# mims-harvard/Raindrop

Measured on AMD Instinct MI355X. Metric: samples/sec fwd+bwd, P19 34-sensor batch=256; % HBM roofline on msg-pass kernel, higher is better.
Workload: dtype f32

## Files before the change

include/raindrop_hip_debug.h:

```cpp
#ifndef RAINDROP_HIP_DEBUG_H
#define RAINDROP_HIP_DEBUG_H

#ifdef __cplusplus
extern "C" {
#endif

void rd_debug_set_stamps(void* device_u64);
void rd_debug_set_rowgemm_stamps(void* device_u64);
void rd_debug_set_attn_stamps(void* device_u64);
void rd_debug_set_gemm_stamps(void* device_u64);
void rd_debug_set_encfuse_stamps(void* device_u64);
void rd_debug_set_head_stamps(void* device_u64);
void rd_debug_set_attnfuse_stamps(void* device_u64);
void rd_debug_ifetch_probe(void* ticks_device_u64, void* scratch_64_floats, void* stream);
void rd_debug_set_splitk_want(int workgroups);

#ifdef __cplusplus
}
#endif
#endif
```

raindrop_amd/csrc/rd_attnfuse.hip:

```cpp
#include <stdlib.h>

#include "rd_common.h"
#include "rd_plan.h"
#include "rd_rng.h"

namespace rd {
namespace {

typedef __bf16 bf8 __attribute__((ext_vector_type(8)));
typedef __bf16 bf4 __attribute__((ext_vector_type(4)));
typedef short sh4 __attribute__((ext_vector_type(4)));
typedef short sh8 __attribute__((ext_vector_type(8)));

constexpr int TS = 64;
constexpr int LDT = TS;
__device__ __forceinline__ int tsw(int row) { return (row & 3) | (((row >> 3) & 1) << 2); }
__device__ __forceinline__ int tofs(int row, int col) { return row * LDT + ((((col >> 3) ^ tsw(row)) & 7) << 3) + (col & 7); }
constexpr int AF_WV = 8, AF_THR = 64 * AF_WV;

struct FAttnArgs {
  const float* x;
  const __bf16* wf;
  const __bf16* wb;
  const float* bias;
  float* out; float* lse;
  const float* dout; const float* ds1; float* dx;
  __bf16* xt; __bf16* dt;
  const int32_t* plan;
  int T, B, D, H, hd;
  float scale, p_drop; uint64_t seed; uint32_t site; const uint64_t* seed_cell;
  int one;
  unsigned long long* stamps;
};
static unsigned long long* g_af_stamps = nullptr;
#define AFSTAMP(i)                                                                                  \
  do {                                                                                              \
    if (a.stamps && blockIdx.x == 0 && threadIdx.x == 0) a.stamps[(i)] = clock64();                 \
  } while (0)

__device__ __forceinline__ float g16_max(float v) {
#define RD_ROR(v, n) __builtin_bit_cast(float, __builtin_amdgcn_update_dpp(0, __builtin_bit_cast(int, v), 0x120 + (n), 0xf, 0xf, false))
  v = fmaxf(v, RD_ROR(v, 8)); v = fmaxf(v, RD_ROR(v, 4)); v = fmaxf(v, RD_ROR(v, 2)); v = fmaxf(v, RD_ROR(v, 1));
  return v;
}
__device__ __forceinline__ float g16_sum(float v) {
  v += RD_ROR(v, 8); v += RD_ROR(v, 4); v += RD_ROR(v, 2); v += RD_ROR(v, 1);
#undef RD_ROR
  return v;
}

__device__ __forceinline__ bf8 frag_n(const __bf16* P, int ld, int row0, int k0, int lane) {
  return *reinterpret_cast<const bf8*>(P + (row0 + (lane & 15)) * ld + k0 + 8 * (lane >> 4));
}
__device__ __forceinline__ bf8 frag_t(const __bf16* P, int ld, int k0, int col0, int lane) {
  const int i = lane & 15, G = lane >> 4;
  const __bf16* src = P + (k0 + 8 * G + (i >> 2)) * ld + col0 + 4 * (i & 3);
  const sh4 lo = __builtin_amdgcn_ds_read_tr16_b64_v4i16((sh4 __attribute__((address_space(3)))*)(src));
  const sh4 hi = __builtin_amdgcn_ds_read_tr16_b64_v4i16((sh4 __attribute__((address_space(3)))*)(src + 4 * ld));
  const sh8 o = {lo[0], lo[1], lo[2], lo[3], hi[0], hi[1], hi[2], hi[3]};
  return __builtin_bit_cast(bf8, o);
}
__device__ __forceinline__ bf8 frag_ns(const __bf16* P, int row0, int k0, int lane) {
  return *reinterpret_cast<const bf8*>(P + tofs(row0 + (lane & 15), k0 + 8 * (lane >> 4)));
}
__device__ __forceinline__ bf8 frag_ts(const __bf16* P, int k0, int col0, int lane) {
  const int i = lane & 15, G = lane >> 4;
  const int row = k0 + 8 * G + (i >> 2), col = col0 + 4 * (i & 3);
  const __bf16* src = P + tofs(row, col);
  const sh4 lo = __builtin_amdgcn_ds_read_tr16_b64_v4i16((sh4 __attribute__((address_space(3)))*)(src));
  const sh4 hi = __builtin_amdgcn_ds_read_tr16_b64_v4i16((sh4 __attribute__((address_space(3)))*)(src + 4 * LDT));
  const sh8 o = {lo[0], lo[1], lo[2], lo[3], hi[0], hi[1], hi[2], hi[3]};
  return __builtin_bit_cast(bf8, o);
}
template <int NT, bool AT, bool BT, bool ASW, bool BSW>
__device__ __forceinline__ void mma_b16(f32x4 (&acc)[NT], const __bf16* Ah, const __bf16* Al, int lda, int a0, const __bf16* Bh,
                                        const __bf16* Bl, int ldb, int b0, int KK, int lane, bool one) {
  auto fa = [&](const __bf16* P, int k0) {
    if (ASW) return AT ? frag_ts(P, k0, a0, lane) : frag_ns(P, a0, k0, lane);
    return AT ? frag_t(P, lda, k0, a0, lane) : frag_n(P, lda, a0, k0, lane);
  };
  auto fb = [&](const __bf16* P, int k0, int j) {
    if (BSW) return BT ? frag_ts(P, k0, b0 + 16 * j, lane) : frag_ns(P, b0 + 16 * j, k0, lane);
    return BT ? frag_t(P, ldb, k0, b0 + 16 * j, lane) : frag_n(P, ldb, b0 + 16 * j, k0, lane);
  };
  if (!one) {
#pragma unroll
    for (int k0 = 0; k0 < KK; k0 += 32) {
      const bf8 ah = fa(Ah, k0);
      const bf8 al = fa(Al, k0);
      bf8 bh[NT], bl[NT];
#pragma unroll
      for (int j = 0; j < NT; ++j) { bh[j] = fb(Bh, k0, j); bl[j] = fb(Bl, k0, j); }
#pragma unroll
      for (int j = 0; j < NT; ++j) acc[j] = __builtin_amdgcn_mfma_f32_16x16x32_bf16(al, bh[j], acc[j], 0, 0, 0);
#pragma unroll
      for (int j = 0; j < NT; ++j) acc[j] = __builtin_amdgcn_mfma_f32_16x16x32_bf16(ah, bl[j], acc[j], 0, 0, 0);
#pragma unroll
      for (int j = 0; j < NT; ++j) acc[j] = __builtin_amdgcn_mfma_f32_16x16x32_bf16(ah, bh[j], acc[j], 0, 0, 0);
    }
  } else {
#pragma unroll
    for (int k0 = 0; k0 < KK; k0 += 32) {
      const bf8 ah = fa(Ah, k0);
#pragma unroll
      for (int j = 0; j < NT; ++j) {
        const bf8 bh = fb(Bh, k0, j);
        acc[j] = __builtin_amdgcn_mfma_f32_16x16x32_bf16(ah, bh, acc[j], 0, 0, 0);
      }
    }
  }
}

__device__ __forceinline__ void split4(const float (&v)[4], bf4& hi, bf4& lo) {
#pragma unroll
  for (int r = 0; r < 4; ++r) { hi[r] = (__bf16)v[r]; lo[r] = (__bf16)(v[r] - (float)hi[r]); }
}
__device__ __forceinline__ void store_t4(__bf16* Ph, __bf16* Pl, int row, int col4, const float (&v)[4]) {
  bf4 hi, lo;
  split4(v, hi, lo);
  const int o = tofs(row, col4);
  *reinterpret_cast<bf4*>(Ph + o) = hi;
  *reinterpret_cast<bf4*>(Pl + o) = lo;
}

__device__ __forceinline__ uint64_t attn_quad(int bh, int T, int q, int key) { return ((uint64_t)bh * T + key) * ((T + 3) >> 2) + (q >> 2); }
__device__ __forceinline__ void attn_keep4(float (&k4)[4], uint64_t seed, uint32_t site, int bh, int T, int q0, int key, float p, float inv_keep) {
  const float4 u = uniform4(seed, site, attn_quad(bh, T, q0, key));
  k4[0] = u.x >= p ? inv_keep : 0.f; k4[1] = u.y >= p ? inv_keep : 0.f;
  k4[2] = u.z >= p ? inv_keep : 0.f; k4[3] = u.w >= p ? inv_keep : 0.f;
}

template <int KCX>
struct XRows { float4 v[(TS * 8 * KCX) / AF_THR]; };

template <int KCX>
__device__ __forceinline__ void x_request(XRows<KCX>& r, const float* x, long row0, int Tv, int D, int tid) {
  constexpr int kq = 8 * KCX, NIT = (TS * kq) / AF_THR;
  static_assert((TS * kq) % AF_THR == 0, "x tile must divide over the workgroup");
#pragma unroll
  for (int it = 0; it < NIT; ++it) {
    const int i = tid + it * AF_THR;
    const int rr = i / kq, k = 4 * (i - rr * kq);
    r.v[it] = *reinterpret_cast<const float4*>(x + (row0 + min(rr, Tv - 1)) * D + min(k, D - 4));
  }
}
template <int KCX>
__device__ __forceinline__ void x_store(const XRows<KCX>& r, __bf16* Xh, __bf16* Xl, int Tv, int D, int tid) {
  constexpr int kq = 8 * KCX, NIT = (TS * kq) / AF_THR, LDX = 32 * KCX + 16;
#pragma unroll
  for (int it = 0; it < NIT; ++it) {
    const int i = tid + it * AF_THR;
    const int rr = i / kq, k = 4 * (i - rr * kq);
    const bool ok = rr < Tv && k < D;
    const float v[4] = {ok ? r.v[it].x : 0.f, ok ? r.v[it].y : 0.f, ok ? r.v[it].z : 0.f, ok ? r.v[it].w : 0.f};
    bf4 hi, lo;
    split4(v, hi, lo);
    *reinterpret_cast<bf4*>(Xh + rr * LDX + k) = hi;
    *reinterpret_cast<bf4*>(Xl + rr * LDX + k) = lo;
  }
}

template <int KCX>
struct QkvPanel { bf8 h[2][KCX], l[2][KCX]; float bs[2]; };

template <int NTH, int KCX>
__device__ __forceinline__ void qkv_request(QkvPanel<KCX>& p, const __bf16* wf_h, const float* bias, int D, int hd, int h, int wave, int lane) {
  constexpr int NCT3 = 3 * NTH;
  static_assert(NCT3 <= 2 * AF_WV, "two column tiles per wave");
#pragma unroll
  for (int s = 0; s < 2; ++s) {
    const int ct = min(wave + AF_WV * s, NCT3 - 1);
    const __bf16* t = wf_h + (size_t)ct * (KCX * 2 * 512) + lane * 8;
#pragma unroll
    for (int kc = 0; kc < KCX; ++kc) {
      p.h[s][kc] = *reinterpret_cast<const bf8*>(t + (kc * 2 + 0) * 512);
      p.l[s][kc] = *reinterpret_cast<const bf8*>(t + (kc * 2 + 1) * 512);
    }
    const int whc = ct / NTH, cl = 16 * (ct - whc * NTH) + (lane & 15);
    p.bs[s] = bias[whc * D + h * hd + min(cl, hd - 1)];
  }
}

template <int NTH, int KCX>
__device__ __forceinline__ void qkv_project(const QkvPanel<KCX>& p, const __bf16* Xh, const __bf16* Xl, int hd, int Tv, __bf16* Tp, int wave,
                                            int lane, bool one) {
  constexpr int NCT3 = 3 * NTH, HDP = 32 * ((16 * NTH + 31) / 32), LDX = 32 * KCX + 16;
  const bool two = wave + AF_WV < NCT3;
  const int aoff = (lane & 15) * LDX + 8 * (lane >> 4);
  f32x4 acc[2][4];
#pragma unroll
  for (int s = 0; s < 2; ++s)
#pragma unroll
    for (int rt = 0; rt < 4; ++rt) acc[s][rt] = (f32x4){0.f, 0.f, 0.f, 0.f};
  if (!one) {
#pragma unroll
    for (int kc = 0; kc < KCX; ++kc) {
      bf8 ah[4], al[4];
#pragma unroll
      for (int rt = 0; rt < 4; ++rt) {
        ah[rt] = *reinterpret_cast<const bf8*>(Xh + rt * 16 * LDX + aoff + kc * 32);
        al[rt] = *reinterpret_cast<const bf8*>(Xl + rt * 16 * LDX + aoff + kc * 32);
      }
#pragma unroll
      for (int s = 0; s < 2; ++s)
#pragma unroll
        for (int rt = 0; rt < 4; ++rt) acc[s][rt] = __builtin_amdgcn_mfma_f32_16x16x32_bf16(al[rt], p.h[s][kc], acc[s][rt], 0, 0, 0);
#pragma unroll
      for (int s = 0; s < 2; ++s)
#pragma unroll
        for (int rt = 0; rt < 4; ++rt) acc[s][rt] = __builtin_amdgcn_mfma_f32_16x16x32_bf16(ah[rt], p.l[s][kc], acc[s][rt], 0, 0, 0);
#pragma unroll
      for (int s = 0; s < 2; ++s)
#pragma unroll
        for (int rt = 0; rt < 4; ++rt) acc[s][rt] = __builtin_amdgcn_mfma_f32_16x16x32_bf16(ah[rt], p.h[s][kc], acc[s][rt], 0, 0, 0);
    }
  } else {
#pragma unroll
    for (int kc = 0; kc < KCX; ++kc) {
#pragma unroll
      for (int rt = 0; rt < 4; ++rt) {
        const bf8 ah = *reinterpret_cast<const bf8*>(Xh + rt * 16 * LDX + aoff + kc * 32);
#pragma unroll
        for (int s = 0; s < 2; ++s) acc[s][rt] = __builtin_amdgcn_mfma_f32_16x16x32_bf16(ah, p.h[s][kc], acc[s][rt], 0, 0, 0);
      }
    }
  }
#pragma unroll
  for (int s = 0; s < 2; ++s) {
    if (s == 1 && !two) break;
    const int ct = wave + AF_WV * s;
    const int whc = ct / NTH, cl = 16 * (ct - whc * NTH) + (lane & 15);
    __bf16* Ph = Tp + (size_t)(whc * 2) * HDP * LDT;
    __bf16* Pl = Ph + (size_t)HDP * LDT;
    const bool cok = cl < hd;
#pragma unroll
    for (int rt = 0; rt < 4; ++rt) {
      const int r0 = 16 * rt + 4 * (lane >> 4);
      float v[4];
#pragma unroll
      for (int r = 0; r < 4; ++r) v[r] = (cok && r0 + r < Tv) ? acc[s][rt][r] + p.bs[s] : 0.f;
      store_t4(Ph, Pl, cl, r0, v);
    }
  }
}

template <int NTH>
__device__ __forceinline__ void zero_pad_rows(__bf16* Tp, int tid) {
  constexpr int HDP = 32 * ((16 * NTH + 31) / 32), PADR = HDP - 16 * NTH;
  if (PADR == 0) return;
  constexpr int Q8 = LDT / 4;
  for (int i = tid; i < 6 * PADR * Q8; i += AF_THR) {
    const int pl = i / (PADR * Q8), rem = i - pl * (PADR * Q8);
    const int rr = rem / Q8, q = rem - rr * Q8;
    bf4 z;
#pragma unroll
    for (int c = 0; c < 4; ++c) z[c] = (__bf16)0.f;
    *reinterpret_cast<bf4*>(Tp + ((size_t)pl * HDP + 16 * NTH + rr) * LDT + 4 * q) = z;
  }
}

template <int NTH, int KCX, bool ONE>
__global__ __launch_bounds__(AF_THR) void k_attn_fwd_fused(FAttnArgs a) {
  extern __shared__ __attribute__((aligned(16))) unsigned char fsm[];
  RD_TOUCH_CODE(ONE ? RD_TL_ATTN_FWD_B : RD_TL_ATTN_FWD);
  constexpr int HDP = 32 * ((16 * NTH + 31) / 32), LDX = 32 * KCX + 16, NA = (NTH + 1) / 2;
  constexpr int LDO = 16 * NTH + 4;
  __bf16* Xh = reinterpret_cast<__bf16*>(fsm);
  __bf16* Xl = Xh + TS * LDX;
  __bf16* Tp = Xl + TS * LDX;
  __bf16 *Qh = Tp, *Ql = Qh + HDP * LDT, *Kh = Ql + HDP * LDT, *Kl = Kh + HDP * LDT, *Vh = Kl + HDP * LDT, *Vl = Vh + HDP * LDT;
  float* mxs = reinterpret_cast<float*>(Vl + HDP * LDT);
  float* sms = mxs + 2 * TS;
  __bf16 *Ph = Qh, *Pl = Ql;
  float* ost = reinterpret_cast<float*>(Kh);
  static_assert(HDP >= TS, "P^T must fit inside the Q^T plane");
  static_assert((size_t)TS * LDO * 4 <= (size_t)2 * HDP * LDT * 2, "output stage must fit inside the K^T planes");
  const int tid = threadIdx.x, lane = tid & 63, wave = __builtin_amdgcn_readfirstlane(tid >> 6), wq = wave & 3, wh = wave >> 2;
  const int b = blockIdx.x;
  const int Tv = __builtin_amdgcn_readfirstlane(a.plan[plan::len_base(a.B) + b]);
  if (Tv <= 0) return;
  const long row0 = __builtin_amdgcn_readfirstlane(a.plan[plan::off_base() + b]);
  uint64_t seedv = a.seed;
  XRows<KCX> xr;
  x_request<KCX>(xr, a.x, row0, Tv, a.D, tid);
  QkvPanel<KCX> pan;
  qkv_request<NTH, KCX>(pan, a.wf, a.bias, a.D, a.hd, 0, wave, lane);
  __builtin_amdgcn_sched_barrier(0);
  if (a.p_drop > 0.f && a.seed_cell) seedv += load_uniform_u64(a.seed_cell);
  zero_pad_rows<NTH>(Tp, tid);
  AFSTAMP(0);
  x_store<KCX>(xr, Xh, Xl, Tv, a.D, tid);
  AFSTAMP(1);
  lds_barrier();
  AFSTAMP(2);
  const float inv_keep = 1.0f / (1.0f - a.p_drop);
  constexpr bool one = ONE;
  const int qr0 = wq * 16 + 4 * (lane >> 4);
  for (int h = 0; h < a.H; ++h) {
    const int bh = b * a.H + h;
    if (h > 0) zero_pad_rows<NTH>(Tp, tid);
    qkv_project<NTH, KCX>(pan, Xh, Xl, a.hd, Tv, Tp, wave, lane, one);
    __builtin_amdgcn_sched_barrier(0);
    {
      const int hn = h + 1 < a.H ? h + 1 : 0;
      qkv_request<NTH, KCX>(pan, a.wf + (size_t)hn * (3 * NTH * KCX * 2 * 512), a.bias, a.D, a.hd, hn, wave, lane);
    }
    __builtin_amdgcn_sched_barrier(0);
    AFSTAMP(3 + 8 * h);
    lds_barrier();
    AFSTAMP(4 + 8 * h);
    float kp[2][4];
#pragma unroll
    for (int j = 0; j < 2; ++j)
      attn_keep4(kp[j], seedv, a.site, bh, a.T, qr0, min(16 * (2 * wh + j) + (lane & 15), a.T - 1), a.p_drop, inv_keep);
    f32x4 s[2];
#pragma unroll
    for (int j = 0; j < 2; ++j) s[j] = (f32x4){0.f, 0.f, 0.f, 0.f};
    mma_b16<2, true, true, true, true>(s, Qh, Ql, LDT, wq * 16, Kh, Kl, LDT, 32 * wh, HDP, lane, one);
    float mx[4] = {-INFINITY, -INFINITY, -INFINITY, -INFINITY};
#pragma unroll
    for (int j = 0; j < 2; ++j) {
      const int key = 16 * (2 * wh + j) + (lane & 15);
      const bool dead = key >= Tv;
#pragma unroll
      for (int r = 0; r < 4; ++r) {
        s[j][r] = dead ? -INFINITY : s[j][r] * a.scale;
        mx[r] = fmaxf(mx[r], s[j][r]);
      }
    }
#pragma unroll
    for (int r = 0; r < 4; ++r) {
      mx[r] = g16_max(mx[r]);
      if ((lane & 15) == 0) mxs[wh * TS + qr0 + r] = mx[r];
    }
    AFSTAMP(5 + 8 * h);
    lds_barrier();
    float m_i[4], rsum[4] = {0.f, 0.f, 0.f, 0.f};
#pragma unroll
    for (int r = 0; r < 4; ++r) m_i[r] = fmaxf(mxs[qr0 + r], mxs[TS + qr0 + r]);
#pragma unroll
    for (int j = 0; j < 2; ++j) {
      const int key = 16 * (2 * wh + j) + (lane & 15);
      float pv[4];
#pragma unroll
      for (int r = 0; r < 4; ++r) {
        const float p = (s[j][r] == -INFINITY) ? 0.f : __expf(s[j][r] - m_i[r]);
        rsum[r] += p;
        pv[r] = p * kp[j][r];
      }
      store_t4(Ph, Pl, key, qr0, pv);
    }
#pragma unroll
    for (int r = 0; r < 4; ++r) {
      rsum[r] = g16_sum(rsum[r]);
      if ((lane & 15) == 0) sms[wh * TS + qr0 + r] = rsum[r];
    }
    AFSTAMP(6 + 8 * h);
    lds_barrier();
    AFSTAMP(7 + 8 * h);
    float l_i[4];
#pragma unroll
    for (int r = 0; r < 4; ++r) l_i[r] = sms[qr0 + r] + sms[TS + qr0 + r];
    const int t0 = wh * NA;
    f32x4 o[NA];
#pragma unroll
    for (int j = 0; j < NA; ++j) o[j] = (f32x4){0.f, 0.f, 0.f, 0.f};
    mma_b16<NA, true, false, true, true>(o, Ph, Pl, LDT, wq * 16, Vh, Vl, LDT, 16 * t0, TS, lane, one);
#pragma unroll
    for (int r = 0; r < 4; ++r) {
      const int q = qr0 + r;
      const float inv = 1.0f / l_i[r];
#pragma unroll
      for (int j = 0; j < NA; ++j)
        if (t0 + j < NTH) ost[q * LDO + 16 * (t0 + j) + (lane & 15)] = o[j][r] * inv;
      if (wh == 0 && (lane & 15) == 0 && q < Tv) a.lse[(long)bh * a.T + q] = m_i[r] + logf(l_i[r]);
    }
    AFSTAMP(8 + 8 * h);
    lds_barrier();
    AFSTAMP(9 + 8 * h);
    {
      const int qpr = a.hd >> 2;
      for (int e = tid; e < Tv * qpr; e += AF_THR) {
        const int q = e / qpr, c4 = e - q * qpr;
        *reinterpret_cast<float4*>(a.out + (row0 + q) * a.D + h * a.hd + 4 * c4) = *reinterpret_cast<const float4*>(ost + q * LDO + 4 * c4);
      }
    }
    lds_barrier();
    AFSTAMP(10 + 8 * h);
  }
}

template <int NTH, int KCX>
constexpr size_t fwd_lds() {
  constexpr int HDP = 32 * ((16 * NTH + 31) / 32), LDX = 32 * KCX + 16;
  return (size_t)2 * TS * LDX * 2 + (size_t)6 * HDP * LDT * 2 + (size_t)4 * TS * 4;
}

template <int NTH>
struct HRegs { float4 v[(4 * NTH + 7) / 8]; unsigned ok; };
template <int NTH>
__device__ __forceinline__ void head_request(HRegs<NTH>& h, const float* base, long ld, int Tv, int hd, int tl) {
  constexpr int NCH = (4 * NTH + 7) / 8;
  const int t = tl >> 3;
  const bool rok = t < Tv;
  const float* src = base + (long)(rok ? t : 0) * ld;
  unsigned ok = 0;
#pragma unroll
  for (int i = 0; i < NCH; ++i) {
    const int c = 4 * ((tl & 7) + 8 * i);
    const bool cok = c < hd;
    h.v[i] = *reinterpret_cast<const float4*>(src + (cok ? c : 0));
    if (rok && cok) ok |= 1u << i;
  }
  h.ok = ok;
}
template <int NTH>
__device__ __forceinline__ void head_mask(HRegs<NTH>& h) {
  constexpr int NCH = (4 * NTH + 7) / 8;
#pragma unroll
  for (int i = 0; i < NCH; ++i)
    if (!((h.ok >> i) & 1u)) h.v[i] = make_float4(0.f, 0.f, 0.f, 0.f);
}

template <int KB>
struct DxPanel { bf8 h[2][KB], l[2][KB]; };

template <int KCX, int KB, int NS>
__device__ __forceinline__ void dx_request(DxPanel<KB>& p, const __bf16* wb_h, int which, int wave, int lane) {
  constexpr int NCT = 2 * KCX;
#pragma unroll
  for (int s = 0; s < NS; ++s) {
    const __bf16* t = wb_h + ((size_t)which * NCT + wave + AF_WV * s) * (KB * 2 * 512) + lane * 8;
#pragma unroll
    for (int kc = 0; kc < KB; ++kc) {
      p.h[s][kc] = *reinterpret_cast<const bf8*>(t + (kc * 2 + 0) * 512);
      p.l[s][kc] = *reinterpret_cast<const bf8*>(t + (kc * 2 + 1) * 512);
    }
  }
}
template <int NTH, int KB, int NS, bool ONE>
__device__ __forceinline__ void dx_mma(f32x4 (&dxa)[2][4], const DxPanel<KB>& p, const __bf16* Tp, int which, int lane) {
  constexpr int HDP = 32 * ((16 * NTH + 31) / 32);
// ... 38 lines not shown
  __builtin_amdgcn_sched_barrier(0);
  dx_mma<NTH, KB, NS, ONE>(dxa, p0, Tp, 2, lane);
  __builtin_amdgcn_sched_barrier(0);
}

template <int NTH, int KCX, bool ONE>
__global__ __launch_bounds__(AF_THR) void k_attn_bwd_fused(FAttnArgs a) {
  extern __shared__ __attribute__((aligned(16))) unsigned char fsm[];
  RD_TOUCH_CODE(ONE ? RD_TL_ATTN_BWD_B : RD_TL_ATTN_BWD);
  constexpr int HDP = 32 * ((16 * NTH + 31) / 32), LDX = 32 * KCX + 16, NA = (NTH + 1) / 2, KB = HDP / 32, LDB = HDP + 16;
  constexpr int NCT = 2 * KCX;
  constexpr int LDS_DX = 32 * KCX + 4;
  __bf16* Xh = reinterpret_cast<__bf16*>(fsm);
  __bf16* Xl = Xh + TS * LDX;
  __bf16 *Ph = Xh, *Pl = Ph + TS * LDT, *Sh = Pl + TS * LDT, *Sl = Sh + TS * LDT;
  float* dxs = reinterpret_cast<float*>(fsm);
  static_assert((size_t)4 * TS * LDT * 2 <= (size_t)2 * TS * LDX * 2, "score planes must fit inside the x planes");
  static_assert((size_t)TS * LDS_DX * 4 <= (size_t)2 * TS * LDX * 2, "dx stage must fit inside the x planes");
  __bf16* Tp = Xl + TS * LDX;
  __bf16 *Qh = Tp, *Ql = Qh + HDP * LDT, *Kh = Ql + HDP * LDT, *Kl = Kh + HDP * LDT, *Vh = Kl + HDP * LDT, *Vl = Vh + HDP * LDT;
  __bf16* Oh = Vl + HDP * LDT;
  __bf16* Ol = Oh + TS * LDB;
  float* lse_s = reinterpret_cast<float*>(Ol + TS * LDB);
  float* dl_s = lse_s + TS;
  const int tid = threadIdx.x, lane = tid & 63, wave = __builtin_amdgcn_readfirstlane(tid >> 6), wq = wave & 3, wh = wave >> 2;
  const int b = blockIdx.x;
  const int Tv = __builtin_amdgcn_readfirstlane(a.plan[plan::len_base(a.B) + b]);
  if (Tv <= 0) return;
  const long row0 = __builtin_amdgcn_readfirstlane(a.plan[plan::off_base() + b]);
  const int g0 = __builtin_amdgcn_readfirstlane(a.plan[plan::coff_base(a.B, a.T) + b]);
  const int ngrp = (Tv + 15) >> 4;
  const bool tail_zero = (g0 + ngrp) == __builtin_amdgcn_readfirstlane(a.plan[plan::coff_base(a.B, a.T) + a.B]) && ((g0 + ngrp) & 1);
  uint64_t seedv = a.seed;
  if (a.p_drop > 0.f && a.seed_cell) seedv += load_uniform_u64(a.seed_cell);
  const float inv_keep = 1.0f / (1.0f - a.p_drop);
  constexpr bool one = ONE;
  f32x4 dxa[2][4];
#pragma unroll
  for (int s = 0; s < 2; ++s)
#pragma unroll
    for (int rt = 0; rt < 4; ++rt) dxa[s][rt] = (f32x4){0.f, 0.f, 0.f, 0.f};
  const bool two = wave + AF_WV < NCT;
  constexpr int NQ = (TS * 8 * KCX + AF_THR - 1) / AF_THR;
  QkvPanel<KCX> pan;
  HRegs<NTH> dov, ov; float lrow;
  head_request<NTH>(dov, a.dout + row0 * a.D, a.D, Tv, a.hd, tid);
  head_request<NTH>(ov, a.out + row0 * a.D, a.D, Tv, a.hd, tid);
  lrow = a.lse[(long)(b * a.H) * a.T + min(tid >> 3, Tv - 1)];
  for (int h = 0; h < a.H; ++h) {
    const int bh = b * a.H + h;
    int tl = tid;
    asm volatile("" : "+v"(tl));
    XRows<KCX> xr;
    x_request<KCX>(xr, a.x, row0, Tv, a.D, tl);
    int lq = lane;
    asm volatile("" : "+v"(lq));
    qkv_request<NTH, KCX>(pan, a.wf + (size_t)h * (3 * NTH * KCX * 2 * 512), a.bias, a.D, a.hd, h, wave, lq);
    AFSTAMP(32 + 16 * h);
    __builtin_amdgcn_sched_barrier(0);
    if (h == 0) zero_pad_rows<NTH>(Tp, tl);
    x_store<KCX>(xr, Xh, Xl, Tv, a.D, tl);
    AFSTAMP(33 + 16 * h);
    lds_barrier();
    AFSTAMP(34 + 16 * h);
    if (h == 0) {
      const int i16 = lq & 15, g2 = (lq >> 4) & 1, sub = lq >> 5;
      const int npair = (ngrp + 1) >> 1;
      for (int t = wave; t < npair * NCT * 2; t += AF_WV) {
        const int plane = t & 1, cj = t >> 1;
        const int pr = cj / NCT, j = cj - pr * NCT;
        const int lg = 2 * pr + sub;
        const __bf16* src = (plane ? Xl : Xh) + (16 * min(lg, ngrp - 1) + 8 * g2 + (i16 >> 2)) * LDX + 16 * j + 4 * (i16 & 3);
        const sh4 lo = __builtin_amdgcn_ds_read_tr16_b64_v4i16((sh4 __attribute__((address_space(3)))*)(src));
        const sh4 hi = __builtin_amdgcn_ds_read_tr16_b64_v4i16((sh4 __attribute__((address_space(3)))*)(src + 4 * LDX));
        const sh8 o = {lo[0], lo[1], lo[2], lo[3], hi[0], hi[1], hi[2], hi[3]};
        const int gg = g0 + lg;
        if (lg < ngrp)
          *reinterpret_cast<sh8*>(a.xt + (((size_t)(gg >> 1) * NCT + j) * 2 + plane) * 512 + (32 * (gg & 1) + 16 * g2 + i16) * 8) = o;
      }
      if (tail_zero) {
        const int gg = g0 + ngrp;
        const sh8 z = {0, 0, 0, 0, 0, 0, 0, 0};
        for (int i = tid; i < NCT * 2 * 32; i += AF_THR) {
          const int slot = i & 31, jp = i >> 5;
          *reinterpret_cast<sh8*>(a.xt + ((size_t)(gg >> 1) * NCT * 2 + jp) * 512 + (32 + slot) * 8) = z;
        }
      }
    }
    {
      constexpr int NCH = (4 * NTH + 7) / 8;
      head_mask<NTH>(dov);
      head_mask<NTH>(ov);
      float d = 0.f;
#pragma unroll
      for (int i = 0; i < NCH; ++i)
        d += (dov.v[i].x * ov.v[i].x + dov.v[i].y * ov.v[i].y) + (dov.v[i].z * ov.v[i].z + dov.v[i].w * ov.v[i].w);
      d += __shfl_xor(d, 1);
      d += __shfl_xor(d, 2);
      d += __shfl_xor(d, 4);
      const int o = (tl >> 3) * LDB + 4 * (tl & 7);
#pragma unroll
      for (int i = 0; i < NCH; ++i) {
        static_assert(32 * NCH == HDP, "8 threads x NCH chunks cover exactly the padded head width (chunks >= hd arrive as zeros)");
        const float v[4] = {dov.v[i].x, dov.v[i].y, dov.v[i].z, dov.v[i].w};
        bf4 hi, lo;
        split4(v, hi, lo);
        *reinterpret_cast<bf4*>(Oh + o + 32 * i) = hi;
        *reinterpret_cast<bf4*>(Ol + o + 32 * i) = lo;
      }
      if ((tl & 7) == 0) { dl_s[tl >> 3] = d; lse_s[tl >> 3] = lrow; }
    }
    __builtin_amdgcn_sched_barrier(0);
    {
      const int hn = h + 1 < a.H ? h + 1 : 0;
// ... 103 lines not shown
      }
    }
    AFSTAMP(44 + 16 * h);
    if (two) { if (one) dx_phase<NTH, KCX, 2, true>(dxa, dp0, Tp, wb_h, wave, ld); else dx_phase<NTH, KCX, 2, false>(dxa, dp0, Tp, wb_h, wave, ld); }
    else { if (one) dx_phase<NTH, KCX, 1, true>(dxa, dp0, Tp, wb_h, wave, ld); else dx_phase<NTH, KCX, 1, false>(dxa, dp0, Tp, wb_h, wave, ld); }
    AFSTAMP(45 + 16 * h);
  }
  float4 r4[NQ];
  {
    const int qpr = a.D >> 2;
#pragma unroll
    for (int i = 0; i < NQ; ++i) {
      const int e = tid + i * AF_THR, q = e / qpr, c4 = e - q * qpr;
      r4[i] = *reinterpret_cast<const float4*>(a.ds1 + (row0 + min(q, Tv - 1)) * a.D + 4 * c4);
    }
  }
  __builtin_amdgcn_sched_barrier(0);
#pragma unroll
  for (int s = 0; s < 2; ++s) {
    if (s == 1 && !two) break;
    const int ct = wave + AF_WV * s;
#pragma unroll
    for (int rt = 0; rt < 4; ++rt)
#pragma unroll
      for (int r = 0; r < 4; ++r) dxs[(16 * rt + 4 * (lane >> 4) + r) * LDS_DX + 16 * ct + (lane & 15)] = dxa[s][rt][r];
  }
  AFSTAMP(64);
  lds_barrier();
  {
    const int qpr = a.D >> 2;
#pragma unroll
    for (int i = 0; i < NQ; ++i) {
      const int e = tid + i * AF_THR, q = e / qpr, c4 = e - q * qpr;
      if (q < Tv) {
        const float4 s4 = *reinterpret_cast<const float4*>(dxs + q * LDS_DX + 4 * c4);
        *reinterpret_cast<float4*>(a.dx + (row0 + q) * a.D + 4 * c4) = make_float4(s4.x + r4[i].x, s4.y + r4[i].y, s4.z + r4[i].z, s4.w + r4[i].w);
      }
    }
  }
  AFSTAMP(65);
}

template <int NTH, int KCX>
constexpr size_t bwd_lds() {
  constexpr int HDP = 32 * ((16 * NTH + 31) / 32), LDX = 32 * KCX + 16, LDB = HDP + 16;
  return (size_t)2 * TS * LDX * 2 + (size_t)6 * HDP * LDT * 2 + (size_t)2 * TS * LDB * 2 + (size_t)2 * TS * 4;
}

constexpr int AF_NTH = 5, AF_KCX = 5;

}

extern "C" void rd_debug_set_attnfuse_stamps(void* p) { g_af_stamps = (unsigned long long*)p; }

bool attnfuse_ok(int T, int D, int H, int hd) {
  const char* e = getenv("RD_ATTN_FUSE");
  const bool enabled = !(e && atoi(e) == 0);
  return enabled && precision() != RD_PREC_FP32 && T <= TS && hd <= 16 * AF_NTH && hd * H == D && (D + 31) / 32 == AF_KCX && (D % 4) == 0 &&
         (hd % 4) == 0 && H >= 1 && H <= 2 && 3 * AF_NTH <= 2 * AF_WV;
}
size_t attnfuse_wf_elems(int H) { return (size_t)H * 3 * AF_NTH * AF_KCX * 2 * 512; }
size_t attnfuse_wb_elems(int H) { return (size_t)H * 3 * (2 * AF_KCX) * ((16 * AF_NTH + 31) / 32) * 2 * 512; }
int attnfuse_split_specs(const float* in_proj_w, int D, int H, int hd, void* wf, void* wb, WsplitSpec* out) {
  constexpr int KB = (16 * AF_NTH + 31) / 32;
  int n = 0;
  for (int h = 0; h < H; ++h)
    for (int which = 0; which < 3; ++which) {
      const float* W = in_proj_w + ((size_t)which * D + (size_t)h * hd) * D;
      out[n++] = WsplitSpec{W, hd, D, 0, (__bf16*)wf + ((size_t)(h * 3 + which) * AF_NTH) * (AF_KCX * 2 * 512)};
      out[n++] = WsplitSpec{W, hd, D, 1, (__bf16*)wb + ((size_t)(h * 3 + which) * (2 * AF_KCX)) * (KB * 2 * 512)};
    }
  return n;
}
int attnfuse_padded_cols(int H) { return 3 * H * 16 * AF_NTH; }
int attnfuse_nth() { return AF_NTH; }

static void fill_args(FAttnArgs& a, const float* x, const void* wf, const void* wb, const float* bias, const int32_t* plan, int T, int B,
                      int D, int H, int hd, float p_drop, uint64_t seed, uint32_t site) {
  a.x = x; a.wf = (const __bf16*)wf; a.wb = (const __bf16*)wb; a.bias = bias; a.plan = plan;
  a.T = T; a.B = B; a.D = D; a.H = H; a.hd = hd;
  a.scale = 1.0f / sqrtf((float)hd); a.p_drop = p_drop; a.seed = seed; a.site = site; a.seed_cell = seed_cell();
  a.one = precision() == RD_PREC_BF16; a.stamps = g_af_stamps;
}

int launch_attn_fused_fwd(const float* x, const void* wf, const float* bias, const int32_t* plan, int T, int B, int D, int H, int hd,
                          float p_drop, uint64_t seed, uint32_t site, float* out, float* lse, hipStream_t st) {
  if (!plan) return fail(RD_EINVAL, "fused attention: needs a token plan");
  FAttnArgs a{};
  fill_args(a, x, wf, nullptr, bias, plan, T, B, D, H, hd, p_drop, seed, site);
  a.out = out; a.lse = lse;
  constexpr size_t lds = fwd_lds<AF_NTH, AF_KCX>();
  if (a.one) { RD_LDS_ATTR((k_attn_fwd_fused<AF_NTH, AF_KCX, true>), lds);
               hipLaunchKernelGGL((k_attn_fwd_fused<AF_NTH, AF_KCX, true>), dim3(B), dim3(AF_THR), lds, st, a); }
  else { RD_LDS_ATTR((k_attn_fwd_fused<AF_NTH, AF_KCX, false>), lds);
         hipLaunchKernelGGL((k_attn_fwd_fused<AF_NTH, AF_KCX, false>), dim3(B), dim3(AF_THR), lds, st, a); }
  return check_launch("k_attn_fwd_fused");
}

int launch_attn_fused_bwd(const float* x, const void* wf, const void* wb, const float* bias, const int32_t* plan, int T, int B, int D, int H,
                          int hd, float p_drop, uint64_t seed, uint32_t site, const float* out, const float* lse, const float* dout,
                          const float* ds1, float* dx, void* xt, void* dt, hipStream_t st) {
  if (!plan) return fail(RD_EINVAL, "fused attention: needs a token plan");
  FAttnArgs a{};
  fill_args(a, x, wf, wb, bias, plan, T, B, D, H, hd, p_drop, seed, site);
  a.out = const_cast<float*>(out); a.lse = const_cast<float*>(lse); a.dout = dout; a.ds1 = ds1; a.dx = dx;
  a.xt = (__bf16*)xt; a.dt = (__bf16*)dt;
  constexpr size_t lds = bwd_lds<AF_NTH, AF_KCX>();
  if (a.one) { RD_LDS_ATTR((k_attn_bwd_fused<AF_NTH, AF_KCX, true>), lds);
               hipLaunchKernelGGL((k_attn_bwd_fused<AF_NTH, AF_KCX, true>), dim3(B), dim3(AF_THR), lds, st, a); }
  else { RD_LDS_ATTR((k_attn_bwd_fused<AF_NTH, AF_KCX, false>), lds);
         hipLaunchKernelGGL((k_attn_bwd_fused<AF_NTH, AF_KCX, false>), dim3(B), dim3(AF_THR), lds, st, a); }
  return check_launch("k_attn_bwd_fused");
}

}
```

raindrop_amd/csrc/rd_touch_gen.h:

```cpp
#pragma once
#define RD_TL_K1_FWD_P19 13056
#define RD_TL_K1_BWD_P19 10368
#define RD_TL_K1_FWD 16640
#define RD_TL_K1_BWD 11648
#define RD_TL_ATTN_FWD 12800
#define RD_TL_ATTN_BWD 26368
#define RD_TL_ATTN_FWD_B 11136
#define RD_TL_ATTN_BWD_B 19968
#define RD_TL_EF_POST_P19L 41856
#define RD_TL_EF_POST_P19L_B 38272
#define RD_TL_EF_POST_P19 41472
#define RD_TL_EF_POST_P19_B 37888
#define RD_TL_EF_POST_P12L 41344
#define RD_TL_EF_POST_P12L_B 37760
#define RD_TL_EF_POST_P12 40960
#define RD_TL_EF_POST_P12_B 37376
#define RD_TL_EF_POST_RTL 53376
#define RD_TL_EF_POST_RTL_B 49792
#define RD_TL_EF_POST_RT 56320
#define RD_TL_EF_POST_RT_B 52736
#define RD_TL_EF_PRE_P19L 43776
#define RD_TL_EF_PRE_P19L_B 40320
#define RD_TL_EF_PRE_P19 43392
#define RD_TL_EF_PRE_P19_B 39936
#define RD_TL_EF_PRE_P12L 43264
#define RD_TL_EF_PRE_P12L_B 39936
#define RD_TL_EF_PRE_P12 42880
#define RD_TL_EF_PRE_P12_B 39552
#define RD_TL_EF_PRE_RTL 59648
#define RD_TL_EF_PRE_RTL_B 55936
#define RD_TL_EF_PRE_RT 59264
#define RD_TL_EF_PRE_RT_B 55552
#define RD_TL_DW 7424
#define RD_TL_DW_REDUCE 9984
#define RD_TL_ADAM 2944
#define RD_TL_ADAM_DEV 3072
#define RD_TL_WSPLIT 5248
#define RD_TL_TWG 10496
#define RD_TL_TWG_ONE 8832
#define RD_TL_HEAD_P19 15616
#define RD_TL_HEAD 17152
#define RD_TL_GEMM 26368
#define RD_TL_GEMM_X3 30080
#define RD_TL_GEMM_PANEL 33024
#define RD_TL_GEMM_PANEL_WIDE 111232
#define RD_TL_GEMM_PANEL_PC 55552
#define RD_TL_ROWGEMM 4480
#define RD_TL_ATTN_FWD_ONE 6144
#define RD_TL_ATTN_BWD_ONE 6528
#define RD_TL_ATTN_FWD_B16 7424
#define RD_TL_ATTN_BWD_DQ 7552
#define RD_TL_ATTN_BWD_DKV 6400
#define RD_TL_ADD_LN_FWD 5632
#define RD_TL_LN_BWD_R 5632
#define RD_TL_LN_BWD_V 6656
```

Measured before the change: 779,500.

## Skip dead row tiles in fused attention forward and add optional per-head split

```diff
diff --git a/include/raindrop_hip_debug.h b/include/raindrop_hip_debug.h
--- a/include/raindrop_hip_debug.h
+++ b/include/raindrop_hip_debug.h
@@ -12,6 +12,7 @@
 void rd_debug_set_encfuse_stamps(void* device_u64);
 void rd_debug_set_head_stamps(void* device_u64);
 void rd_debug_set_attnfuse_stamps(void* device_u64);
+void rd_debug_set_attnfuse_wg_stamps(void* device_u64);
 void rd_debug_ifetch_probe(void* ticks_device_u64, void* scratch_64_floats, void* stream);
 void rd_debug_set_splitk_want(int workgroups);
 
diff --git a/raindrop_amd/csrc/rd_attnfuse.hip b/raindrop_amd/csrc/rd_attnfuse.hip
--- a/raindrop_amd/csrc/rd_attnfuse.hip
+++ b/raindrop_amd/csrc/rd_attnfuse.hip
@@ -30,9 +30,13 @@
   int T, B, D, H, hd;
   float scale, p_drop; uint64_t seed; uint32_t site; const uint64_t* seed_cell;
   int one;
+  int split_len;
+  int tile_skip;
   unsigned long long* stamps;
+  unsigned long long* wgst;
 };
 static unsigned long long* g_af_stamps = nullptr;
+static unsigned long long* g_af_wgst = nullptr;
 #define AFSTAMP(i)                                                                                  \
   do {                                                                                              \
     if (a.stamps && blockIdx.x == 0 && threadIdx.x == 0) a.stamps[(i)] = clock64();                 \
@@ -74,7 +78,7 @@
 }
 template <int NT, bool AT, bool BT, bool ASW, bool BSW>
 __device__ __forceinline__ void mma_b16(f32x4 (&acc)[NT], const __bf16* Ah, const __bf16* Al, int lda, int a0, const __bf16* Bh,
-                                        const __bf16* Bl, int ldb, int b0, int KK, int lane, bool one) {
+                                        const __bf16* Bl, int ldb, int b0, int KK, int lane, bool one, int K0 = 0) {
   auto fa = [&](const __bf16* P, int k0) {
     if (ASW) return AT ? frag_ts(P, k0, a0, lane) : frag_ns(P, a0, k0, lane);
     return AT ? frag_t(P, lda, k0, a0, lane) : frag_n(P, lda, a0, k0, lane);
@@ -85,7 +89,7 @@
   };
   if (!one) {
 #pragma unroll
-    for (int k0 = 0; k0 < KK; k0 += 32) {
+    for (int k0 = K0; k0 < KK; k0 += 32) {
       const bf8 ah = fa(Ah, k0);
       const bf8 al = fa(Al, k0);
       bf8 bh[NT], bl[NT];
@@ -100,7 +104,7 @@
     }
   } else {
 #pragma unroll
-    for (int k0 = 0; k0 < KK; k0 += 32) {
+    for (int k0 = K0; k0 < KK; k0 += 32) {
       const bf8 ah = fa(Ah, k0);
 #pragma unroll
       for (int j = 0; j < NT; ++j) {
@@ -134,21 +138,23 @@
 struct XRows { float4 v[(TS * 8 * KCX) / AF_THR]; };
 
 template <int KCX>
-__device__ __forceinline__ void x_request(XRows<KCX>& r, const float* x, long row0, int Tv, int D, int tid) {
+__device__ __forceinline__ void x_request(XRows<KCX>& r, const float* x, long row0, int Tv, int D, int tid, int ngrp) {
   constexpr int kq = 8 * KCX, NIT = (TS * kq) / AF_THR;
   static_assert((TS * kq) % AF_THR == 0, "x tile must divide over the workgroup");
 #pragma unroll
   for (int it = 0; it < NIT; ++it) {
+    if ((it * AF_THR) / kq >= 16 * ngrp) break;
     const int i = tid + it * AF_THR;
     const int rr = i / kq, k = 4 * (i - rr * kq);
     r.v[it] = *reinterpret_cast<const float4*>(x + (row0 + min(rr, Tv - 1)) * D + min(k, D - 4));
   }
 }
 template <int KCX>
-__device__ __forceinline__ void x_store(const XRows<KCX>& r, __bf16* Xh, __bf16* Xl, int Tv, int D, int tid) {
+__device__ __forceinline__ void x_store(const XRows<KCX>& r, __bf16* Xh, __bf16* Xl, int Tv, int D, int tid, int ngrp) {
   constexpr int kq = 8 * KCX, NIT = (TS * kq) / AF_THR, LDX = 32 * KCX + 16;
 #pragma unroll
   for (int it = 0; it < NIT; ++it) {
+    if ((it * AF_THR) / kq >= 16 * ngrp) break;
     const int i = tid + it * AF_THR;
     const int rr = i / kq, k = 4 * (i - rr * kq);
     const bool ok = rr < Tv && k < D;
@@ -181,10 +187,11 @@
   }
 }
 
-template <int NTH, int KCX>
+template <int NTH, int KCX, int NG = 4>
 __device__ __forceinline__ void qkv_project(const QkvPanel<KCX>& p, const __bf16* Xh, const __bf16* Xl, int hd, int Tv, __bf16* Tp, int wave,
                                             int lane, bool one) {
-  constexpr int NCT3 = 3 * NTH, HDP = 32 * ((16 * NTH + 31) / 32), LDX = 32 * KCX + 16;
+  constexpr int NCT3 = 3 * NTH, HDP = 32 * ((16 * NTH + 31) / 32), LDX = 32 * KCX + 16, NGS = 2 * ((NG + 1) / 2);
+  static_assert(NG >= 1 && NG <= 4, "row tiles of a sample");
   const bool two = wave + AF_WV < NCT3;
   const int aoff = (lane & 15) * LDX + 8 * (lane >> 4);
   f32x4 acc[2][4];
@@ -197,28 +204,28 @@
     for (int kc = 0; kc < KCX; ++kc) {
       bf8 ah[4], al[4];
 #pragma unroll
-      for (int rt = 0; rt < 4; ++rt) {
+      for (int rt = 0; rt < NG; ++rt) {
         ah[rt] = *reinterpret_cast<const bf8*>(Xh + rt * 16 * LDX + aoff + kc * 32);
         al[rt] = *reinterpret_cast<const bf8*>(Xl + rt * 16 * LDX + aoff + kc * 32);
       }
 #pragma unroll
       for (int s = 0; s < 2; ++s)
 #pragma unroll
-        for (int rt = 0; rt < 4; ++rt) acc[s][rt] = __builtin_amdgcn_mfma_f32_16x16x32_bf16(al[rt], p.h[s][kc], acc[s][rt], 0, 0, 0);
+        for (int rt = 0; rt < NG; ++rt) acc[s][rt] = __builtin_amdgcn_mfma_f32_16x16x32_bf16(al[rt], p.h[s][kc], acc[s][rt], 0, 0, 0);
 #pragma unroll
       for (int s = 0; s < 2; ++s)
 #pragma unroll
-        for (int rt = 0; rt < 4; ++rt) acc[s][rt] = __builtin_amdgcn_mfma_f32_16x16x32_bf16(ah[rt], p.l[s][kc], acc[s][rt], 0, 0, 0);
+        for (int rt = 0; rt < NG; ++rt) acc[s][rt] = __builtin_amdgcn_mfma_f32_16x16x32_bf16(ah[rt], p.l[s][kc], acc[s][rt], 0, 0, 0);
 #pragma unroll
       for (int s = 0; s < 2; ++s)
 #pragma unroll
-        for (int rt = 0; rt < 4; ++rt) acc[s][rt] = __builtin_amdgcn_mfma_f32_16x16x32_bf16(ah[rt], p.h[s][kc], acc[s][rt], 0, 0, 0);
+        for (int rt = 0; rt < NG; ++rt) acc[s][rt] = __builtin_amdgcn_mfma_f32_16x16x32_bf16(ah[rt], p.h[s][kc], acc[s][rt], 0, 0, 0);
     }
   } else {
 #pragma unroll
     for (int kc = 0; kc < KCX; ++kc) {
 #pragma unroll
-      for (int rt = 0; rt < 4; ++rt) {
+      for (int rt = 0; rt < NG; ++rt) {
         const bf8 ah = *reinterpret_cast<const bf8*>(Xh + rt * 16 * LDX + aoff + kc * 32);
 #pragma unroll
         for (int s = 0; s < 2; ++s) acc[s][rt] = __builtin_amdgcn_mfma_f32_16x16x32_bf16(ah, p.h[s][kc], acc[s][rt], 0, 0, 0);
@@ -234,7 +241,7 @@
     __bf16* Pl = Ph + (size_t)HDP * LDT;
     const bool cok = cl < hd;
 #pragma unroll
-    for (int rt = 0; rt < 4; ++rt) {
+    for (int rt = 0; rt < NGS; ++rt) {
       const int r0 = 16 * rt + 4 * (lane >> 4);
       float v[4];
 #pragma unroll
@@ -276,33 +283,48 @@
   static_assert(HDP >= TS, "P^T must fit inside the Q^T plane");
   static_assert((size_t)TS * LDO * 4 <= (size_t)2 * HDP * LDT * 2, "output stage must fit inside the K^T planes");
   const int tid = threadIdx.x, lane = tid & 63, wave = __builtin_amdgcn_readfirstlane(tid >> 6), wq = wave & 3, wh = wave >> 2;
-  const int b = blockIdx.x;
+  int b = blockIdx.x, h0 = 0, h1 = a.H;
+  if (a.split_len >= 0) {
+    const int nL = __builtin_amdgcn_readfirstlane(a.plan[plan::cnt_base(a.B) + a.split_len]);
+    const int w = blockIdx.x;
+    if (w < a.H * nL) { b = a.H == 2 ? w >> 1 : w / a.H; h0 = w - b * a.H; h1 = h0 + 1; }
+    else { b = w - (a.H - 1) * nL; if (b >= a.B) return; }
+  }
   const int Tv = __builtin_amdgcn_readfirstlane(a.plan[plan::len_base(a.B) + b]);
   if (Tv <= 0) return;
   const long row0 = __builtin_amdgcn_readfirstlane(a.plan[plan::off_base() + b]);
+  const int ngrp = a.tile_skip ? (Tv + 15) >> 4 : 4;
+  if (a.wgst && tid == 0) a.wgst[2 * blockIdx.x] = wall_clock64();
   uint64_t seedv = a.seed;
   XRows<KCX> xr;
-  x_request<KCX>(xr, a.x, row0, Tv, a.D, tid);
+  x_request<KCX>(xr, a.x, row0, Tv, a.D, tid, ngrp);
   QkvPanel<KCX> pan;
-  qkv_request<NTH, KCX>(pan, a.wf, a.bias, a.D, a.hd, 0, wave, lane);
+  qkv_request<NTH, KCX>(pan, a.wf + (size_t)h0 * (3 * NTH * KCX * 2 * 512), a.bias, a.D, a.hd, h0, wave, lane);
   __builtin_amdgcn_sched_barrier(0);
   if (a.p_drop > 0.f && a.seed_cell) seedv += load_uniform_u64(a.seed_cell);
   zero_pad_rows<NTH>(Tp, tid);
   AFSTAMP(0);
-  x_store<KCX>(xr, Xh, Xl, Tv, a.D, tid);
+  x_store<KCX>(xr, Xh, Xl, Tv, a.D, tid, ngrp);
   AFSTAMP(1);
   lds_barrier();
   AFSTAMP(2);
   const float inv_keep = 1.0f / (1.0f - a.p_drop);
   constexpr bool one = ONE;
   const int qr0 = wq * 16 + 4 * (lane >> 4);
-  for (int h = 0; h < a.H; ++h) {
+  const bool qlive = wq < ngrp;
+  const bool klive = 2 * wh < ngrp;
+  for (int h = h0; h < h1; ++h) {
     const int bh = b * a.H + h;
-    if (h > 0) zero_pad_rows<NTH>(Tp, tid);
-    qkv_project<NTH, KCX>(pan, Xh, Xl, a.hd, Tv, Tp, wave, lane, one);
+    if (h > h0) zero_pad_rows<NTH>(Tp, tid);
+    switch (ngrp) {
+      case 1: qkv_project<NTH, KCX, 1>(pan, Xh, Xl, a.hd, Tv, Tp, wave, lane, one); break;
+      case 2: qkv_project<NTH, KCX, 2>(pan, Xh, Xl, a.hd, Tv, Tp, wave, lane, one); break;
+      case 3: qkv_project<NTH, KCX, 3>(pan, Xh, Xl, a.hd, Tv, Tp, wave, lane, one); break;
+      default: qkv_project<NTH, KCX, 4>(pan, Xh, Xl, a.hd, Tv, Tp, wave, lane, one); break;
+    }
     __builtin_amdgcn_sched_barrier(0);
     {
-      const int hn = h + 1 < a.H ? h + 1 : 0;
+      const int hn = h + 1 < h1 ? h + 1 : h0;
       qkv_request<NTH, KCX>(pan, a.wf + (size_t)hn * (3 * NTH * KCX * 2 * 512), a.bias, a.D, a.hd, hn, wave, lane);
     }
     __builtin_amdgcn_sched_barrier(0);
@@ -310,70 +332,78 @@
     lds_barrier();
     AFSTAMP(4 + 8 * h);
     float kp[2][4];
-#pragma unroll
-    for (int j = 0; j < 2; ++j)
-      attn_keep4(kp[j], seedv, a.site, bh, a.T, qr0, min(16 * (2 * wh + j) + (lane & 15), a.T - 1), a.p_drop, inv_keep);
     f32x4 s[2];
 #pragma unroll
     for (int j = 0; j < 2; ++j) s[j] = (f32x4){0.f, 0.f, 0.f, 0.f};
-    mma_b16<2, true, true, true, true>(s, Qh, Ql, LDT, wq * 16, Kh, Kl, LDT, 32 * wh, HDP, lane, one);
-    float mx[4] = {-INFINITY, -INFINITY, -INFINITY, -INFINITY};
-#pragma unroll
-    for (int j = 0; j < 2; ++j) {
-      const int key = 16 * (2 * wh + j) + (lane & 15);
-      const bool dead = key >= Tv;
+    if (qlive) {
+#pragma unroll
+      for (int j = 0; j < 2; ++j)
+        attn_keep4(kp[j], seedv, a.site, bh, a.T, qr0, min(16 * (2 * wh + j) + (lane & 15), a.T - 1), a.p_drop, inv_keep);
+      if (klive) mma_b16<2, true, true, true, true>(s, Qh, Ql, LDT, wq * 16, Kh, Kl, LDT, 32 * wh, HDP, lane, one);
+      float mx[4] = {-INFINITY, -INFINITY, -INFINITY, -INFINITY};
+#pragma unroll
+      for (int j = 0; j < 2; ++j) {
+        const int key = 16 * (2 * wh + j) + (lane & 15);
+        const bool dead = key >= Tv;
+#pragma unroll
+        for (int r = 0; r < 4; ++r) {
+          s[j][r] = dead ? -INFINITY : s[j][r] * a.scale;
+          mx[r] = fmaxf(mx[r], s[j][r]);
+        }
+      }
 #pragma unroll
       for (int r = 0; r < 4; ++r) {
-        s[j][r] = dead ? -INFINITY : s[j][r] * a.scale;
-        mx[r] = fmaxf(mx[r], s[j][r]);
-      }
-    }
-#pragma unroll
-    for (int r = 0; r < 4; ++r) {
-      mx[r] = g16_max(mx[r]);
-      if ((lane & 15) == 0) mxs[wh * TS + qr0 + r] = mx[r];
+        mx[r] = g16_max(mx[r]);
+        if ((lane & 15) == 0) mxs[wh * TS + qr0 + r] = mx[r];
+      }
     }
     AFSTAMP(5 + 8 * h);
     lds_barrier();
-    float m_i[4], rsum[4] = {0.f, 0.f, 0.f, 0.f};
-#pragma unroll
-    for (int r = 0; r < 4; ++r) m_i[r] = fmaxf(mxs[qr0 + r], mxs[TS + qr0 + r]);
-#pragma unroll
-    for (int j = 0; j < 2; ++j) {
-      const int key = 16 * (2 * wh + j) + (lane & 15);
-      float pv[4];
+    float m_i[4] = {0.f, 0.f, 0.f, 0.f};
+    if (qlive) {
+      float rsum[4] = {0.f, 0.f, 0.f, 0.f};
+#pragma unroll
+      for (int r = 0; r < 4; ++r) m_i[r] = fmaxf(mxs[qr0 + r], mxs[TS + qr0 + r]);
+#pragma unroll
+      for (int j = 0; j < 2; ++j) {
+        const int key = 16 * (2 * wh + j) + (lane & 15);
+        float pv[4];
+#pragma unroll
+        for (int r = 0; r < 4; ++r) {
+          const float p = (s[j][r] == -INFINITY) ? 0.f : __expf(s[j][r] - m_i[r]);
+          rsum[r] += p;
+          pv[r] = p * kp[j][r];
+        }
+        store_t4(Ph, Pl, key, qr0, pv);
+      }
 #pragma unroll
       for (int r = 0; r < 4; ++r) {
-        const float p = (s[j][r] == -INFINITY) ? 0.f : __expf(s[j][r] - m_i[r]);
-        rsum[r] += p;
-        pv[r] = p * kp[j][r];
-      }
-      store_t4(Ph, Pl, key, qr0, pv);
-    }
-#pragma unroll
-    for (int r = 0; r < 4; ++r) {
-      rsum[r] = g16_sum(rsum[r]);
-      if ((lane & 15) == 0) sms[wh * TS + qr0 + r] = rsum[r];
+        rsum[r] = g16_sum(rsum[r]);
+        if ((lane & 15) == 0) sms[wh * TS + qr0 + r] = rsum[r];
+      }
     }
     AFSTAMP(6 + 8 * h);
     lds_barrier();
     AFSTAMP(7 + 8 * h);
-    float l_i[4];
-#pragma unroll
-    for (int r = 0; r < 4; ++r) l_i[r] = sms[qr0 + r] + sms[TS + qr0 + r];
-    const int t0 = wh * NA;
-    f32x4 o[NA];
-#pragma unroll
-    for (int j = 0; j < NA; ++j) o[j] = (f32x4){0.f, 0.f, 0.f, 0.f};
-    mma_b16<NA, true, false, true, true>(o, Ph, Pl, LDT, wq * 16, Vh, Vl, LDT, 16 * t0, TS, lane, one);
-#pragma unroll
-    for (int r = 0; r < 4; ++r) {
-      const int q = qr0 + r;
-      const float inv = 1.0f / l_i[r];
-#pragma unroll
-      for (int j = 0; j < NA; ++j)
-        if (t0 + j < NTH) ost[q * LDO + 16 * (t0 + j) + (lane & 15)] = o[j][r] * inv;
-      if (wh == 0 && (lane & 15) == 0 && q < Tv) a.lse[(long)bh * a.T + q] = m_i[r] + logf(l_i[r]);
+    if (qlive) {
+      float l_i[4];
+#pragma unroll
+      for (int r = 0; r < 4; ++r) l_i[r] = sms[qr0 + r] + sms[TS + qr0 + r];
+      const int t0 = wh * NA;
+      f32x4 o[NA];
+#pragma unroll
+      for (int j = 0; j < NA; ++j) o[j] = (f32x4){0.f, 0.f, 0.f, 0.f};
+      mma_b16<NA, true, false, true, true>(o, Ph, Pl, LDT, wq * 16, Vh, Vl, LDT, 16 * t0, 32, lane, one);
+      if (ngrp > 2) mma_b16<NA, true, false, true, true>(o, Ph, Pl, LDT, wq * 16, Vh, Vl, LDT, 16 * t0, TS, lane, one, 32);
+#pragma unroll
+      for (int r = 0; r < 4; ++r) {
+        const int q = qr0 + r;
+        const float inv = 1.0f / l_i[r];
+#pragma unroll
+        for (int j = 0; j < NA; ++j)
+          if (t0 + j < NTH) ost[q * LDO + 16 * (t0 + j) + (lane & 15)] = o[j][r] * inv;
+        if (wh == 0 && (lane & 15) == 0 && q < Tv) a.lse[(long)bh * a.T + q] = m_i[r] + logf(l_i[r]);
+      }
     }
     AFSTAMP(8 + 8 * h);
     lds_barrier();
@@ -388,6 +418,7 @@
     lds_barrier();
     AFSTAMP(10 + 8 * h);
   }
+  if (a.wgst && tid == 0) a.wgst[2 * blockIdx.x + 1] = wall_clock64();
 }
 
 template <int NTH, int KCX>
@@ -532,14 +563,14 @@
     int tl = tid;
     asm volatile("" : "+v"(tl));
     XRows<KCX> xr;
-    x_request<KCX>(xr, a.x, row0, Tv, a.D, tl);
+    x_request<KCX>(xr, a.x, row0, Tv, a.D, tl, 4);
     int lq = lane;
     asm volatile("" : "+v"(lq));
     qkv_request<NTH, KCX>(pan, a.wf + (size_t)h * (3 * NTH * KCX * 2 * 512), a.bias, a.D, a.hd, h, wave, lq);
     AFSTAMP(32 + 16 * h);
     __builtin_amdgcn_sched_barrier(0);
     if (h == 0) zero_pad_rows<NTH>(Tp, tl);
-    x_store<KCX>(xr, Xh, Xl, Tv, a.D, tl);
+    x_store<KCX>(xr, Xh, Xl, Tv, a.D, tl, 4);
     AFSTAMP(33 + 16 * h);
     lds_barrier();
     AFSTAMP(34 + 16 * h);
@@ -749,6 +780,7 @@
 }
 
 extern "C" void rd_debug_set_attnfuse_stamps(void* p) { g_af_stamps = (unsigned long long*)p; }
+extern "C" void rd_debug_set_attnfuse_wg_stamps(void* p) { g_af_wgst = (unsigned long long*)p; }
 
 bool attnfuse_ok(int T, int D, int H, int hd) {
   const char* e = getenv("RD_ATTN_FUSE");
@@ -772,12 +804,24 @@
 int attnfuse_padded_cols(int H) { return 3 * H * 16 * AF_NTH; }
 int attnfuse_nth() { return AF_NTH; }
 
+constexpr int AF_SPLIT_LEN = 32;
+static int attnfuse_split_len(int T, int H) {
+  const char* e = getenv("RD_ATTN_HEAD_SPLIT");
+  if (!(e && atoi(e) != 0) || H < 2) return -1;
+  const char* l = getenv("RD_ATTN_SPLIT_LEN");
+  int L = l ? atoi(l) : AF_SPLIT_LEN;
+  if (L < 0) L = 0;
+  return L >= T ? -1 : L;
+}
+static int attnfuse_tile_skip() { const char* e = getenv("RD_ATTN_TILE_SKIP"); return !(e && atoi(e) == 0); }
+
 static void fill_args(FAttnArgs& a, const float* x, const void* wf, const void* wb, const float* bias, const int32_t* plan, int T, int B,
                       int D, int H, int hd, float p_drop, uint64_t seed, uint32_t site) {
   a.x = x; a.wf = (const __bf16*)wf; a.wb = (const __bf16*)wb; a.bias = bias; a.plan = plan;
   a.T = T; a.B = B; a.D = D; a.H = H; a.hd = hd;
   a.scale = 1.0f / sqrtf((float)hd); a.p_drop = p_drop; a.seed = seed; a.site = site; a.seed_cell = seed_cell();
-  a.one = precision() == RD_PREC_BF16; a.stamps = g_af_stamps;
+  a.one = precision() == RD_PREC_BF16; a.stamps = g_af_stamps; a.wgst = nullptr;
+  a.split_len = -1; a.tile_skip = 1;
 }
 
 int launch_attn_fused_fwd(const float* x, const void* wf, const float* bias, const int32_t* plan, int T, int B, int D, int H, int hd,
@@ -785,12 +829,14 @@
   if (!plan) return fail(RD_EINVAL, "fused attention: needs a token plan");
   FAttnArgs a{};
   fill_args(a, x, wf, nullptr, bias, plan, T, B, D, H, hd, p_drop, seed, site);
-  a.out = out; a.lse = lse;
+  a.out = out; a.lse = lse; a.wgst = g_af_wgst;
+  a.split_len = attnfuse_split_len(T, H); a.tile_skip = attnfuse_tile_skip();
+  const dim3 grid(a.split_len >= 0 ? H * B : B);
   constexpr size_t lds = fwd_lds<AF_NTH, AF_KCX>();
   if (a.one) { RD_LDS_ATTR((k_attn_fwd_fused<AF_NTH, AF_KCX, true>), lds);
-               hipLaunchKernelGGL((k_attn_fwd_fused<AF_NTH, AF_KCX, true>), dim3(B), dim3(AF_THR), lds, st, a); }
+               hipLaunchKernelGGL((k_attn_fwd_fused<AF_NTH, AF_KCX, true>), grid, dim3(AF_THR), lds, st, a); }
   else { RD_LDS_ATTR((k_attn_fwd_fused<AF_NTH, AF_KCX, false>), lds);
-         hipLaunchKernelGGL((k_attn_fwd_fused<AF_NTH, AF_KCX, false>), dim3(B), dim3(AF_THR), lds, st, a); }
+         hipLaunchKernelGGL((k_attn_fwd_fused<AF_NTH, AF_KCX, false>), grid, dim3(AF_THR), lds, st, a); }
   return check_launch("k_attn_fwd_fused");
 }
 
diff --git a/raindrop_amd/csrc/rd_touch_gen.h b/raindrop_amd/csrc/rd_touch_gen.h
--- a/raindrop_amd/csrc/rd_touch_gen.h
+++ b/raindrop_amd/csrc/rd_touch_gen.h
@@ -3,9 +3,9 @@
 #define RD_TL_K1_BWD_P19 10368
 #define RD_TL_K1_FWD 16640
 #define RD_TL_K1_BWD 11648
-#define RD_TL_ATTN_FWD 12800
+#define RD_TL_ATTN_FWD 19456
 #define RD_TL_ATTN_BWD 26368
-#define RD_TL_ATTN_FWD_B 11136
+#define RD_TL_ATTN_FWD_B 16512
 #define RD_TL_ATTN_BWD_B 19968
 #define RD_TL_EF_POST_P19L 41856
 #define RD_TL_EF_POST_P19L_B 38272
```

New measurement: 781,900, median of 3. About the same (+0.3%).
